# cvxopt/smcp

Measured on AMD Instinct MI355X. Metric: Newton KKT solves/sec, higher is better.
Workload: dtype f64; 1 GPU; synth50k nested block-arrow SDP n=50000, 8073 cliques, m=100; kktsolver=chol, n=50000, cliques=8073, m=100, blkval_doubles=2493568, update_doubles=10689536, parallelism=single

## Files before the change

smcp_amd/csrc/capi.hip:

```cpp
#include <hip/hip_runtime.h>
#include <memory>
#include <unordered_map>

#include <algorithm>
#include <chrono>
#include <cstdio>
#include <cstring>
#include <map>
#include <new>
#include <atomic>
#include <thread>
#include <type_traits>
#include <vector>

#include "../../include/smcp_amd.h"
#include "context.hpp"
#include "switches.hpp"
#include "front_generic.hip"
#include "front_mfma.hip"
#include "front_large.hip"
#include "front_inv.hip"
#include "front_n16.hip"
#include "front_fam.hip"
#include "front_fam2.hip"
#include "front_lfsp.hip"
#include "front_leafgram.hip"
#include "front_famt.hip"
#include "front_flow.hip"
#include "front_mrc.hip"
#include "front_edm.hip"

using namespace smcp;

#define HIPCHK(x)                                                                        \
  do {                                                                                   \
    hipError_t e_ = (x);                                                                 \
    if (e_ != hipSuccess) {                                                              \
      fprintf(stderr, "smcp_amd: HIP error %s at %s:%d\n", hipGetErrorString(e_), __FILE__, __LINE__); \
      return SMCP_EHIP;                                                                  \
    }                                                                                    \
  } while (0)

namespace {

enum {
  KID_chol_level = 0, KID_llt_level, KID_pinv_level, KID_gather_level, KID_completion_all,
  KID_hess_up_level, KID_hess_down_level, KID_hess_down_inv_all, KID_hess_up_inv_level, KID_scale_an,
  KID_factor_yaa, KID_trsm_fwd_level, KID_trsm_bwd_level, KID_amap, KID_aadj, KID_scatter_constraints,
  KID_dense_potrf, KID_dense_potrs, KID_vec_axpby, KID_axpby, KID_reduce_cliques, KID_reduce_final,
  KID_hess_up_mfma, KID_hess_down_mfma, KID_chol_mfma, KID_pinv_mfma, KID_prep_lk,
  KID_hess_up_mfma_hbm, KID_hess_down_mfma_hbm, KID_chol_mfma_hbm, KID_pinv_mfma_hbm,
  KID_gram_partial, KID_gram_reduce, KID_hess_up_pad,
  KID_lf_assemble, KID_lf_clear_upd, KID_lf_up1, KID_lf_up2, KID_lf_up3, KID_lf_down1, KID_lf_down2, KID_lf_down3,
  KID_lf_pinv1, KID_lf_pinv2, KID_lf_diag, KID_lf_chol_panel, KID_lf_chol_trail, KID_lf_pack_upd,
  KID_lf_prep_s, KID_lf_prep_row, KID_lf_prep_k, KID_factor_yaa_lds,
  KID_factor_inverse, KID_hess_down_inv_mfma, KID_hess_down_inv_mfma_hbm, KID_hess_up_inv_mfma, KID_hess_up_inv_mfma_hbm,
  KID_completion_mfma, KID_completion_mfma_hbm, KID_lf_copy_an, KID_lf_ri_an, KID_lf_dinv1, KID_lf_dinv2,
  KID_lf_uinv1, KID_lf_uinv2, KID_lf_completion, KID_hess_up_n16, KID_llt_mfma, KID_llt_mfma_hbm, KID_lf_llt,
  KID_hess_up_fam, KID_qr_rmul, KID_qr_dots, KID_qr_comb, KID_qr_small, KID_fam2_prep, KID_mid_chol, KID_lf_diag_inv, KID_lfsp_up, KID_lfsp_prep, KID_leaf_gram, KID_leaf_tables, KID_fam_sparse, KID_gram_diag128, KID_lf_assemble_lds, KID_fam_terms, KID_famt_prep, KID_lf_assemble_lds_dyn, KID_lf_zsp, KID_fam_terms_grp, KID_lf_assemble_fz, KID_factor_inverse_lds, KID_chol_flow,
  KID_mrc_diag, KID_mrc_rank, KID_mrc_reduce, KID_mrc_factor, KID_cut_signs, KID_cut_weights,
  KID_edm_rank, KID_edm_reduce, KID_edm_factor, KID_edm_dense,
  KID_COUNT
};
const char* const KID_NAMES[KID_COUNT] = {
  "k_chol_level", "k_llt_level", "k_pinv_level", "k_gather_level", "k_completion_all",
  "k_hess_up_level", "k_hess_down_level", "k_hess_down_inv_all", "k_hess_up_inv_level", "k_scale_an",
  "k_factor_yaa", "k_trsm_fwd_level", "k_trsm_bwd_level", "k_amap", "k_aadj", "k_scatter_constraints",
  "k_dense_potrf", "k_dense_potrs", "k_vec_axpby", "k_axpby", "k_reduce_cliques", "k_reduce_final",
  "k_hess_up_mfma<true>", "k_hess_down_mfma<true>", "k_chol_mfma<true>", "k_pinv_mfma<true>", "k_prep_lk",
  "k_hess_up_mfma<false>", "k_hess_down_mfma<false>", "k_chol_mfma<false>", "k_pinv_mfma<false>",
  "k_gram_partial", "k_gram_reduce", "k_hess_up_pad",
  "k_lf_assemble", "k_lf_clear_upd", "k_lf_up1", "k_lf_up2", "k_lf_up3", "k_lf_down1", "k_lf_down2", "k_lf_down3",
  "k_lf_pinv1", "k_lf_pinv2", "k_lf_diag", "k_lf_chol_panel", "k_lf_chol_trail", "k_lf_pack_upd",
  "k_lf_prep_s", "k_lf_prep_row", "k_lf_prep_k", "k_factor_yaa_lds",
  "k_factor_inverse", "k_hess_down_inv_mfma<true>", "k_hess_down_inv_mfma<false>", "k_hess_up_inv_mfma<true>",
  "k_hess_up_inv_mfma<false>", "k_completion_mfma<true>", "k_completion_mfma<false>", "k_lf_copy_an", "k_lf_ri_an",
  "k_lf_dinv1", "k_lf_dinv2", "k_lf_uinv1", "k_lf_uinv2", "k_lf_completion", "k_hess_up_n16",
  "k_llt_mfma<true>", "k_llt_mfma<false>", "k_lf_llt", "k_hess_up_fam",
  "k_stack_trsm", "k_stack_dots", "k_stack_comb", "k_qr_small", "k_fam2_prep", "k_mid_chol", "k_lf_diag_inv", "k_lfsp_up", "k_lfsp_prep", "k_leaf_pairs", "k_leaf_tables", "k_fam_sparse", "k_gram_diag128", "k_lf_assemble_lds", "k_fam_terms", "k_famt_prep", "k_lf_assemble_lds_dyn", "k_lf_zsp", "k_fam_terms_grp", "k_lf_assemble_fz", "k_factor_inverse_lds", "k_chol_flow",
  "k_mrc_diag", "k_mrc_rank", "k_mrc_reduce", "k_mrc_factor", "k_cut_signs", "k_cut_weights",
  "k_edm_rank", "k_edm_reduce", "k_edm_factor", "k_edm_dense"};

inline void note_launch(csp_ctx* c, int kid) {
  const hipError_t e = hipGetLastError();
  if (e != hipSuccess && !c->launch_err) {
    c->launch_err = (int)e;
    fprintf(stderr, "smcp_amd: launch of %s failed: %s\n", (kid >= 0 && kid < KID_COUNT) ? KID_NAMES[kid] : "?", hipGetErrorString(e));
  }
}
inline hipError_t end_call(csp_ctx* c) {
  hipError_t e = hipGetLastError();
  if (e == hipSuccess && c->launch_err) e = c->launch_err > 0 ? (hipError_t)c->launch_err : hipErrorLaunchFailure;
  c->launch_err = 0;
  return e;
}

__global__ void k_race_spin(long long ticks) {
  const long long t0 = wall_clock64();
  for (int it = 0; it < (1 << 22) && wall_clock64() - t0 < ticks; ++it) __builtin_amdgcn_s_sleep(8);
}
struct RaceInject {
  std::atomic<uint64_t> state{0};
  std::atomic<int64_t> injected{0};
  std::atomic<int> max_us{200};
  std::atomic<int> drop_joins{0};
  bool on() const { return state.load(std::memory_order_relaxed) != 0; }
  void seed(uint64_t s) { state.store(s ? (s * 0x9E3779B97F4A7C15ull) | 1ull : 0ull); }
  uint64_t next() {
    uint64_t x = state.load(std::memory_order_relaxed);
    x ^= x << 13; x ^= x >> 7; x ^= x << 17;
    state.store(x | 1ull, std::memory_order_relaxed);
    return x;
  }
};
inline RaceInject& race_inject() {
  static RaceInject r;
  static const bool init = [] { const char* e = sw_str("SMCP_RACE"); if (e && atoll(e) > 0) r.seed((uint64_t)atoll(e)); return true; }();
  (void)init;
  return r;
}
inline void race_delay(hipStream_t s, bool always = true) {
  RaceInject& r = race_inject();
  if (!r.on()) return;
  const uint64_t x = r.next();
  if (!always && (x >> 40) % 4 != 0) return;
  const long long us = 5 + (long long)((x >> 16) % (uint64_t)std::max(1, r.max_us.load(std::memory_order_relaxed) - 4));
  hipLaunchKernelGGL(k_race_spin, dim3(1), dim3(64), 0, s, us * 100);
  r.injected.fetch_add(1, std::memory_order_relaxed);
}

inline unsigned sync_event_flags() {
  static int sys = -1;
  if (sys < 0) { const char* e = sw_str("SMCP_EVENT_SYSFENCE"); sys = (e && e[0] == '1') ? 1 : 0; }
  return sys ? hipEventDisableTiming : (hipEventDisableTiming | hipEventReleaseToDevice);
}
struct Fork {
  csp_ctx* c; hipStream_t main; hipStream_t s; int which; bool on;
  static bool enabled() {
    static int e = -1;
    if (e < 0) { const char* v = sw_str("SMCP_FORK"); e = (v && v[0] == '0') ? 0 : 1; }
    return e == 1 && !trace_on_early();
  }
  static bool trace_on_early() { static const bool t = [] { const char* e = sw_str("SMCP_TRACE"); return e && e[0] == '1'; }(); return t; }
  Fork(csp_ctx* c_, hipStream_t st, int which_) : c(c_), main(st), s(st), which(which_), on(false) {
    if (!enabled()) return;
    if (!c->aux_fork && hipEventCreateWithFlags(&c->aux_fork, sync_event_flags()) != hipSuccess) { c->aux_fork = nullptr; return; }
    if (!c->aux_stream[which]) {
      static int prio = -2;
      if (prio == -2) { const char* e = sw_str("SMCP_AUX_PRIO"); prio = (e && e[0] == '0') ? 0 : 1; }
      int lo = 0, hi = 0;
      hipError_t rc = hipErrorUnknown;
      static int prio1 = -2;
      if (prio1 == -2) { const char* e = sw_str("SMCP_AUX_PRIO1"); prio1 = (e && e[0] == '0') ? 0 : 1; }
      if (which == 0 && prio && hipDeviceGetStreamPriorityRange(&lo, &hi) == hipSuccess && hi < lo)
        rc = hipStreamCreateWithPriority(&c->aux_stream[which], hipStreamNonBlocking, hi);
      if (which == 1 && prio1 && hipDeviceGetStreamPriorityRange(&lo, &hi) == hipSuccess && hi < lo)
        rc = hipStreamCreateWithPriority(&c->aux_stream[which], hipStreamNonBlocking, lo);
      if (rc != hipSuccess) rc = hipStreamCreateWithFlags(&c->aux_stream[which], hipStreamNonBlocking);
      if (rc != hipSuccess) { c->aux_stream[which] = nullptr; return; }
    }
    if (!c->aux_join[which] && hipEventCreateWithFlags(&c->aux_join[which], sync_event_flags()) != hipSuccess) { c->aux_join[which] = nullptr; return; }
    if (hipEventRecord(c->aux_fork, main) != hipSuccess) return;
    if (hipStreamWaitEvent(c->aux_stream[which], c->aux_fork, 0) != hipSuccess) return;
    s = c->aux_stream[which];
    on = true;
    if (race_inject().on()) {
      if (race_inject().drop_joins.load(std::memory_order_relaxed)) {
        hipLaunchKernelGGL(k_race_spin, dim3(1), dim3(64), 0, s, (long long)race_inject().max_us.load() * 100);
      } else race_delay((race_inject().next() >> 33) & 1 ? s : main);
    }
  }
  void join() {
    if (!on) return;
    on = false;
    if (race_inject().on() && ((race_inject().next() >> 33) & 1)) race_delay(s);
    if (race_inject().drop_joins.load(std::memory_order_relaxed)) { (void)hipEventRecord(c->aux_join[which], s); return; }
    if (hipEventRecord(c->aux_join[which], s) != hipSuccess || hipStreamWaitEvent(main, c->aux_join[which], 0) != hipSuccess)
      (void)hipStreamSynchronize(s);
  }
  ~Fork() { join(); }
};

inline bool trace_on() {
  static int t = -1;
  if (t < 0) { const char* e = sw_str("SMCP_TRACE"); t = (e && e[0] == '1') ? 1 : 0; }
  return t == 1;
}
inline void trace_launch(int kid, dim3 grid, dim3 block, size_t lds, hipStream_t st, bool before) {
  if (before) fprintf(stderr, "launch %s grid (%u,%u,%u) block %u lds %zu\n", KID_NAMES[kid], grid.x, grid.y, grid.z, block.x, lds);
  else (void)hipStreamSynchronize(st);
}
template <class K, class... A>
inline void launch_lds(csp_ctx* c, int kid, K kern, dim3 grid, dim3 block, size_t lds, hipStream_t st, A... args) {
  if (trace_on()) trace_launch(kid, grid, block, lds, st, true);
  Profiler& P = c->prof;
  const bool timed = P.want(kid);
  if (timed) (void)hipEventRecord(P.next(), st);
  race_delay(st, false);
  hipLaunchKernelGGL(kern, grid, block, lds, st, args...);
  note_launch(c, kid);
  if (trace_on()) trace_launch(kid, grid, block, lds, st, false);
  if (timed) {
    (void)hipEventRecord(P.next(), st);
    P.kids.push_back(kid);
  }
}
template <class K, class... A>
inline void launch(csp_ctx* c, int kid, K kern, dim3 grid, dim3 block, hipStream_t st, A... args) {
  if (trace_on()) trace_launch(kid, grid, block, 0, st, true);
  Profiler& P = c->prof;
  const bool timed = P.want(kid);
  if (timed) (void)hipEventRecord(P.next(), st);
  race_delay(st, false);
  hipLaunchKernelGGL(kern, grid, block, 0, st, args...);
  note_launch(c, kid);
  if (trace_on()) trace_launch(kid, grid, block, 0, st, false);
  if (timed) {
    (void)hipEventRecord(P.next(), st);
    P.kids.push_back(kid);
  }
}

template <class F>
void run_threads(int nth, F work) {
  if (nth <= 1) { work(0); return; }
  std::vector<std::thread> pool;
  int started = 0;
  try {
    for (; started < nth; ++started) pool.emplace_back(work, started);
  } catch (...) {
  }
  for (int tix = started; tix < nth; ++tix) work(tix);
  for (auto& th : pool) th.join();
}
// ... 1025 lines not shown
                          c->D.kc_ij && a0.ymode == 2 && a0.ysc && c->D.fam_maxterms <= FAMT_TCAP / 2 &&
                          c->D.cnnz <= (int64_t)4 * c->S.nsn * std::max<int64_t>(1, c->D.m);
  if (groups_on || fgroups_on) a0.chskip = groups_on && fgroups_on ? c->D.both_skip : (groups_on ? c->D.lfsp_skip : c->D.famt_skip);
  c->fz_live = false;
  {
    static int fzenv = -1;
    if (fzenv < 0) { const char* e = sw_str("SMCP_FZ"); fzenv = (e && e[0] == '0') ? 0 : 1; }
    bool want = fzenv && sparse && (set == 0 || (set == 1 && c->fz_set1_ok)) && lev_lo == 0 && lev_hi < 0 && !fgroups_on && c->D.fz_ok && !famt_disabled() && !fam2_disabled() &&
                c->D.lg_request && c->D.kc_ij && a0.ymode == 2 && a0.ysc && famt_terms_ok(c->D) &&
                c->D.cnnz <= (int64_t)4 * c->S.nsn * std::max<int64_t>(1, c->D.m) && !use_generic(c) && use_large() && c->D.gp_tptr;
    int famlevels = 0, nofill = 0;
    if (want) {
      for (int64_t l = 0; l < c->S.nlev; ++l)
        for_level_classes(c, l, a0, [&](bool lds, MfmaArgs a, int cnt, size_t, int) {
          if (lds && a.nS > 0 && a.level > 0) ++famlevels;
          if (!lds && (size_t)a.level < c->fz_levels.size() && c->fz_levels[(size_t)a.level] && !(a.nchmax > 0 && lf_assemble_fills(c, a, cnt, nrhs, true))) { want = false; ++nofill; }
        }, set);
      if (famlevels != 1) want = false;
    }
    if (want) { a0.fz_on = 1; a0.fz_no = c->D.fz_no; }
    static int occ = -1;
    if (occ < 0) occ = sw_on("SMCP_OCC", 0);
    if (occ && sparse)
      fprintf(stderr, "fz: want %d famlevels %d nofill %d nlev %d (env %d set %d lev %d..%d fgroups %d fz_ok %d famt_off %d fam2_off %d lg_request %d kc_ij %d ymode %d ysc %d maxterms %d cnnz %lld nsn %lld m %lld generic %d nrhs %d)\n",
              (int)want, famlevels, nofill, (int)c->S.nlev, fzenv, set, (int)lev_lo, (int)lev_hi, (int)fgroups_on, (int)c->D.fz_ok, (int)famt_disabled(), (int)fam2_disabled(), (int)c->D.lg_request,
              c->D.kc_ij != nullptr, a0.ymode, a0.ysc != nullptr, (int)c->D.fam_maxterms, (long long)c->D.cnnz, (long long)c->S.nsn, (long long)c->D.m, (int)use_generic(c), nrhs);
  }
  auto dense_input_on = [&](MfmaArgs& a, int cnt, double* Ub, int nr, hipStream_t s) {
    if (!sparse) return;
    for (int r0 = 0; r0 < nr; r0 += 65535) {
      MfmaArgs af = a;
      af.kc_j0 = a.kc_j0 + r0;
      const int64_t pan = (int64_t)(a.nnmax + a.namax) * a.nnmax;
      const int nz = (int)std::max<int64_t>(1, std::min<int64_t>(std::min<int64_t>(a.nnmax, 64), pan / 16384));
      launch(c, KID_scatter_constraints, k_panel_fill, dim3(cnt, std::min(65535, nr - r0), nz), dim3(256), s, af, Ub + (int64_t)r0 * ldu, ldu);
    }
    a.kc_ptr = nullptr;
  };
  auto dense_input = [&](MfmaArgs& a, int cnt) { dense_input_on(a, cnt, U, nrhs, st); };
  for (int64_t l = lev_lo; l < (lev_hi < 0 ? c->S.nlev : lev_hi); ++l) {
    for_level_classes(c, l, a0, [&](bool lds, MfmaArgs a, int cnt, size_t bytes, int thr) {
      static int fam_minrhs = -1;
      if (fam_minrhs < 0) { const char* e = sw_str("SMCP_FAM_MINRHS"); fam_minrhs = e ? atoi(e) : 1; }
      if (lds && a.nS > 0 && (sparse || nrhs >= fam_minrhs)) {
        const int nS = a.nS;
        a.nS = 0;
        if (a.level > 0) {
          MfmaArgs af = a;
          af.t.lev = a.t.lev + (cnt - nS);
          if (fgroups_on && (size_t)l < c->famt_grp.size() && c->famt_grp[(size_t)l].ngroups > 0) {
            af.grp_ptr = c->famt_grp[(size_t)l].ptr; af.grp_list = c->famt_grp[(size_t)l].list; af.famt_ngrp = c->famt_grp[(size_t)l].ngroups;
          }
          if (!try_fam(c, af, nS, nrhs, U, ldu, st)) {
            fprintf(stderr, "smcp_amd: family kernel not launchable (LDS budget or attribute)\n");
            if (!c->launch_err) c->launch_err = -1;
          }
        }
        cnt -= nS;
        if (cnt == 0) return;
      }
      int g = rhs_groups(cnt, nrhs, lds ? 2048 : 1024);
      if (lds) {
        hipStream_t ls = st;
        static int oldk = -1;
        if (oldk < 0) { const char* e = sw_str("SMCP_OLDLDS"); oldk = (e && e[0] == '1') ? 1 : 0; }
        size_t pbytes = (size_t)pad_layout(a.nnmax, a.namax, a.nchmax, a.panmax, a.pkmax, a.plansum).total * sizeof(double);
        if (!oldk && try_n16(c, a, cnt, nrhs, U, ldu, ls)) {
        } else if (!oldk && pbytes <= LDS_LIMIT) {
          dense_input_on(a, cnt, U, nrhs, ls);
          launch_lds(c, KID_hess_up_pad, k_hess_up_pad, dim3(cnt, g), dim3(pbytes > 48 * 1024 ? 512 : 256), pbytes, ls, a, U, ldu);
        } else {
          dense_input_on(a, cnt, U, nrhs, ls);
          launch_lds(c, KID_hess_up_mfma, k_hess_up_mfma<true>, dim3(cnt, g), dim3(thr), bytes, ls, a, U, ldu);
        }
      } else if (use_large() && c->D.gp_tptr) {
        {
          const csp_ctx::LfspGroups* grp = groups_on && (size_t)l < c->lfsp_grp.size() && c->lfsp_grp[(size_t)l].ngroups > 0 ? &c->lfsp_grp[(size_t)l] : nullptr;
          if (sparse && try_lfsp(c, a, cnt, nrhs, U, ldu, st, grp)) return;
          if (grp) {
            fprintf(stderr, "smcp_amd: sparse-input sweep of a grouped level not launchable\n");
            if (!c->launch_err) c->launch_err = -1;
          }
        }
        static int split_min = -1;
        if (split_min < 0) { const char* e = sw_str("SMCP_RHS_SPLIT"); split_min = e ? atoi(e) : 16; }
        static int parts = -1;
        if (parts < 0) { const char* e = sw_str("SMCP_RHS_PARTS"); parts = (e && e[0] == '3') ? 3 : 2; }
        const int ncu_split = c->D.ncu;
        static int dynsplit = -1;
        if (dynsplit < 0) { const char* e = sw_str("SMCP_ALDS_DYN"); const char* f = sw_str("SMCP_RHS_SPLIT_DYN"); dynsplit = ((e && e[0] == '0') || (f && f[0] == '1')) ? 1 : 0; }
        if (dynsplit && split_min > 0 && a.nchmax > 0 && nrhs >= split_min && (int64_t)cnt * nrhs > ncu_split && Fork::enabled()) {
          auto part = [&](int r0, int nr, hipStream_t s) {
            MfmaArgs ap = a;
            ap.nrhs = nr;
            ap.t.upd += (int64_t)r0 * a.t.updlen;
            ap.t.updp += (int64_t)r0 * a.t.updplen;
            ap.t.tmp += (int64_t)r0 * a.t.tmplen;
            ap.kc_j0 = a.kc_j0 + r0;
            dense_input_on(ap, cnt, U + (int64_t)r0 * ldu, nr, s);
            lf_up(c, ap, cnt, nr, U + (int64_t)r0 * ldu, ldu, s);
          };
          if (parts == 3 && nrhs >= 3) {
            const int h1 = nrhs / 3, h2 = (2 * nrhs) / 3;
            Fork f0(c, st, 0);
            part(h2, nrhs - h2, f0.s);
            Fork f1(c, st, 1);
            part(h1, h2 - h1, f1.s);
            part(0, h1, st);
            return;
          }
          const int h = nrhs / 2;
          Fork f(c, st, 0);
          part(h, nrhs - h, f.s);
          part(0, h, st);
          return;
        }
        static int zsp = -1;
        if (zsp < 0) { const char* e = sw_str("SMCP_ZSP"); zsp = (e && e[0] == '0') ? 0 : 1; }
        if (zsp && sparse && c->D.kc_sorted && a.nchmax == 0 && a.namax == 0 && lf_sym_split(a.nnmin) && a.nnmax <= LF_ZSP_MAXNN) {
          const int ntN = tiles64(a.nnmax);
          launch_lds(c, KID_lf_zsp, k_lf_zsp, dim3(a.nnmax, cnt, nrhs), dim3(256), (size_t)a.nnmax * sizeof(double), st, a, U, ldu);
          LAUNCH_PD(c, KID_lf_up2, k_lf_up2, dim3(umax1(ntN * (ntN + 1) / 2), cnt, nrhs), dim3(256), st, a, U, ldu);
          return;
        }
        const bool fzlev = c->fz_live && (size_t)a.level < c->fz_levels.size() && c->fz_levels[(size_t)a.level];
        if (sparse && a.nchmax > 0 && lf_assemble_fills(c, a, cnt, nrhs, fzlev)) {
          lf_up(c, a, cnt, nrhs, U, ldu, st, true);
          return;
        }
        dense_input(a, cnt);
        if (yroot && a.namax == 0 && a.nnmax <= ROOT_FUSED_MAXNN && root_fused()) {
          if (a.nchmax > 0) lf_assemble(c, a, cnt, nrhs, U, ldu, 0, st, true);
          const int ntN = tiles64(a.nnmax);
          LAUNCH_PD(c, KID_lf_up1, k_lf_root1, dim3(umax1(ntN * ntN), cnt, nrhs), dim3(256), st, a, U, ldu, yroot);
          return;
        }
        lf_up(c, a, cnt, nrhs, U, ldu, st);
      }
      else { dense_input(a, cnt); launch_lds(c, KID_hess_up_mfma_hbm, k_hess_up_mfma<false>, dim3(cnt, nrhs), dim3(thr), 0, st, a, U, ldu); }
    }, set);
  }
}
void gather_set(csp_ctx* c, int set, const double* x, int64_t ldx, int nrhs, double* updbase, hipStream_t st) {
  TreeArgs a = tree_args(c);
  const LevelSet& LS = c->sets[set];
  for (int64_t l = c->S.nlev - 1; l >= 0; --l) {
    const LevelClass& L = LS.lvl[l];
    const int cnt = (int)(L.nI + L.nII);
    if (!cnt) continue;
    a.lev = LS.lev2 + LS.off[l];
    launch(c, KID_gather_level, k_gather_level, dim3(cnt, nrhs, gather_parts(std::max(L.namaxI, L.namaxII), (int64_t)cnt * nrhs, c->D.ncu)), dim3(NT), st, a, x, ldx, updbase);
  }
}
void hess_down_fast(csp_ctx* c, double* U, int nrhs, int64_t ldu, const double* ysc, int ymode, hipStream_t st, int set = 0,
                    const double* yroot = nullptr) {
  MfmaArgs a0 = mfma_args(c, ysc, ymode, nrhs);
  for (int64_t l = c->S.nlev - 1; l >= 0; --l)
    for_level_classes(c, l, a0, [&](bool lds, MfmaArgs a, int cnt, size_t bytes, int thr) {
      int g = rhs_groups(cnt, nrhs, lds ? 2048 : 1024);
      if (lds) {
        static int dw = -1;
        if (dw < 0) { const char* e = sw_str("SMCP_DOWN_W"); dw = (e && e[0] == '0') ? 0 : 1; }
        if (dw && ymode == 0 && a.nnmax <= 16 && a.namax <= 64 && a.nnmax >= 1) {
          const int gw = rhs_groups((cnt + 3) / 4, nrhs, 4096);
          const dim3 grid((cnt + 3) / 4, gw), blk(256);
          switch ((std::max(a.namax, 1) + 15) / 16) {
            case 1: launch(c, KID_hess_down_mfma, k_hess_down_w<1>, grid, blk, st, a, U, ldu, cnt); break;
            case 2: launch(c, KID_hess_down_mfma, k_hess_down_w<2>, grid, blk, st, a, U, ldu, cnt); break;
            case 3: launch(c, KID_hess_down_mfma, k_hess_down_w<3>, grid, blk, st, a, U, ldu, cnt); break;
            default: launch(c, KID_hess_down_mfma, k_hess_down_w<4>, grid, blk, st, a, U, ldu, cnt); break;
          }
        } else
        if (ymode == 0) {
          const size_t b0 = (size_t)mfma_lds_doubles_for(WK_DOWN0, a.nnmax, a.namax) * sizeof(double);
          launch_lds(c, KID_hess_down_mfma, k_hess_down_mfma<true, WK_DOWN0>, dim3(cnt, g), dim3(b0 > 48 * 1024 ? 512 : 256), b0, st, a, U, ldu);
        } else
        launch_lds(c, KID_hess_down_mfma, k_hess_down_mfma<true>, dim3(cnt, g), dim3(thr), bytes, st, a, U, ldu);
      }
      else if (use_large() && yroot && a.namax == 0 && a.nnmax <= ROOT_FUSED_MAXNN && root_fused() && c->D.gp_tptr) {
        const int ntN = tiles64(a.nnmax);
        LAUNCH_PD(c, KID_lf_down3, k_lf_root2, dim3(umax1(ntN * (ntN + 1) / 2), cnt, nrhs), dim3(256), st, a, U, ldu, yroot);
      }
      else if (use_large() && (ymode == 0 || ymode == 3 || ymode == 2)) {
        if (ymode && a.namax) {
          const int mtA = tiles64(a.namax), ntN = tiles64(a.nnmax);
          LAUNCH_PD(c, KID_lf_ri_an, k_lf_ri_an, dim3(umax1(mtA * ntN), cnt, nrhs), dim3(256), st, a, U, ldu, ymode == 2 ? 1 : 0);
          launch(c, KID_lf_copy_an, k_lf_copy_an, dim3(umax1(std::min(64, (a.namax * a.nnmax + 255) / 256)), cnt, nrhs), dim3(256), st, a, U, ldu, 0);
        }
        MfmaArgs a2 = a;
        a2.ymode = 0; a2.ysc = nullptr;
        lf_down(c, a2, cnt, nrhs, U, ldu, st);
      }
      else launch_lds(c, KID_hess_down_mfma_hbm, k_hess_down_mfma<false>, dim3(cnt, nrhs), dim3(thr), 0, st, a, U, ldu);
    }, set);
}

void lf_factor_inverse(csp_ctx* c, const MfmaArgs& a, int cnt, hipStream_t st) {
  dim3 blk(256);
  for (int ib = 0; ib < a.namax; ib += LB) {
    launch_lds(c, KID_lf_diag, k_lf_diag, dim3(cnt), diag_blk(), LF_DIAG_LDS, st, a, (double*)nullptr, c->D.fac, 4, ib, 0);
    if (ib > 0) launch(c, KID_lf_prep_s, k_lf_prep_s, dim3(umax1(tiles64(ib)), cnt), blk, st, a, (const double*)c->D.fac, c->D.faci, ib, 4);
    launch(c, KID_lf_prep_row, k_lf_prep_row, dim3(umax1(tiles64(ib) + 1), cnt), blk, st, a, (const double*)c->D.fac, c->D.faci, ib, 4, 0);
  }
}

inline hipError_t zero_flag(csp_ctx* c, hipStream_t st) {
  const bool skip = c->lazy_status && c->flags_clean;
  c->flags_clean = false;
  return skip ? hipSuccess : hipMemsetAsync(c->D.info, 0, sizeof(int) * c->ntrial, st);
}
void complete_fac(csp_ctx* c, hipStream_t st) {
  if (!c->D.fac_partial) return;
  c->D.fac_partial = false;
  MfmaArgs a0 = mfma_args(c, nullptr, 0, 1);
  for_level_classes(c, 0, a0, [&](bool lds, MfmaArgs am, int cnt, size_t, int) {
    if (!lds || !am.namax || am.nS <= 0) return;
    am.t.lev = am.t.lev + (cnt - am.nS);
    const size_t bytes = ((size_t)padld(am.namax) * am.namax + 256 + 8) * sizeof(double);
    launch_lds(c, KID_factor_yaa_lds, k_factor_yaa_lds, dim3(am.nS), dim3(fact_threads(am, 256, 2)), bytes, st, am, (const double*)c->D.yaa, c->D.fac);
  });
}
int prepare_yaa(csp_ctx* c, const double* Y, bool need_fac, hipStream_t st, bool need_inv, bool allow_partial) {
  TreeArgs a = tree_args(c);
  const bool nocache = cache_off();
  if (need_inv) need_fac = true;
  if (need_fac && !allow_partial && c->D.fac_partial && c->D.fac_tag == Y && Y && !nocache) complete_fac(c, st);
  if (nocache || c->D.yaa_tag != Y || !Y) {
    gather_all(c, Y, 0, 1, c->D.yaa, st);
    c->D.yaa_tag = Y;
    c->D.fac_tag = c->D.faci_tag = nullptr;
    c->D.part_valid = false;
    if (Y) fp_record(c, 2, Y, st);
  } else if (int rc = fp_check(c, 2, Y, st)) return rc;
  const bool fast = !use_generic(c) && use_large();
  if (need_fac && c->D.fac_tag != Y) {
    if (fast) {
      MfmaArgs a0 = mfma_args(c, nullptr, 0, 1);
      for_all_large(c, a0, [&](MfmaArgs am, int cnt) {
        if (am.namax) launch(c, KID_axpby, k_copy_upd_blocks, dim3(cnt, umax1(std::min(64, (am.namax * am.namax + 1023) / 1024))), dim3(256), st,
                             am.t, (const double*)c->D.yaa, c->D.fac);
      });
      {
        Fork fl(c, st, 0);
        for_all_large(c, a0, [&](MfmaArgs am, int cnt) { if (am.namax) lf_factor_yaa(c, am, cnt, c->D.fac, fl.s); });
        Fork fs(c, st, 1);
        int turn = 0;
        for (int64_t l = 0; l < c->S.nlev; ++l)
          for_level_classes(c, l, a0, [&](bool lds, MfmaArgs am, int cnt, size_t, int) {
            if (!lds) return;
            size_t bytes = ((size_t)padld(am.namax) * am.namax + 256 + 8) * sizeof(double);
            if (am.namax) launch_lds(c, KID_factor_yaa_lds, k_factor_yaa_lds, dim3(cnt), dim3(fact_threads(am, 256, 2)), bytes, (turn++ & 1) ? fs.s : st, am, (const double*)c->D.yaa, c->D.fac);
          });
      }
    } else {
      launch(c, KID_factor_yaa, k_factor_yaa, dim3((int)c->S.nsn), dim3(NT), st, a, c->D.yaa, c->D.fac);
    }
    c->D.fac_tag = Y;
    c->D.fac_partial = false;
    c->D.faci_tag = nullptr;
    c->D.fac_gen++;
  }
  if (need_inv && c->D.faci_tag != Y) {
    if (fast) {
      a.lev = c->D.lev3idx;
      MfmaArgs a0 = mfma_args(c, nullptr, 0, 1);
      static const bool rd = sw_on("SMCP_FACI_LDS", true);
      bool all_lds = rd;
      if (rd)
        for (int64_t l = 0; l < c->S.nlev; ++l)
          for_level_classes(c, l, a0, [&](bool lds, MfmaArgs am, int, size_t, int) { if (lds && am.namax > 64) all_lds = false; });
      if (!c->D.nI_total) {
      } else if (!all_lds) {
        launch(c, KID_factor_inverse, k_factor_inverse, dim3((int)c->D.nI_total), dim3(256), st, a, (const double*)c->D.fac, c->D.faci);
      } else {
        for (int64_t l = 0; l < c->S.nlev; ++l)
          for_level_classes(c, l, a0, [&](bool lds, MfmaArgs am, int cnt, size_t, int) {
            if (!lds || !am.namax) return;
            if (am.namax <= 32)
              launch_lds(c, KID_factor_inverse_lds, k_factor_inverse_lds<33>, dim3(cnt), dim3(128), (2 * 33 * 32 + 256) * sizeof(double), st, am, (const double*)c->D.fac, c->D.faci);
            else
              launch_lds(c, KID_factor_inverse_lds, k_factor_inverse_lds<65>, dim3(cnt), dim3(256), (2 * 65 * 64 + 1024) * sizeof(double), st, am, (const double*)c->D.fac, c->D.faci);
          });
      }
      for_all_large(c, a0, [&](MfmaArgs am, int cnt) { if (am.namax) lf_factor_inverse(c, am, cnt, st); });
    } else {
      a.lev = c->D.levidx;
      launch(c, KID_factor_inverse, k_factor_inverse, dim3((int)c->S.nsn), dim3(256), st, a, (const double*)c->D.fac, c->D.faci);
    }
    c->D.faci_tag = Y;
  }
  return 0;
}

constexpr size_t INV_STATIC_LDS = 16 * 128 * sizeof(double);
constexpr int LF_INV_MIN_NN = 24;

void hess_down_inv_fast(csp_ctx* c, const double* L, double* U, int nrhs, int64_t ldu, int ymode, hipStream_t st) {
  gather_all(c, U, ldu, nrhs, c->D.upd, st);
  MfmaArgs a0 = mfma_args(c, c->D.faci, ymode, nrhs);
  a0.LK = L;
  dim3 blk(256);
  for (int64_t l = 0; l < c->S.nlev; ++l)
    for_level_classes(c, l, a0, [&](bool lds, MfmaArgs a, int cnt, size_t bytes, int thr) {
      if (lds) {
        int g = rhs_groups(cnt, nrhs, 2048);
        launch_lds(c, KID_hess_down_inv_mfma, k_hess_down_inv_mfma<true>, dim3(cnt, g), dim3(thr), bytes, st, a, U, ldu);
      } else if (!use_large()) {
        launch_lds(c, KID_hess_down_inv_mfma_hbm, k_hess_down_inv_mfma<false>, dim3(cnt, nrhs), dim3(thr), 0, st, a, U, ldu);
      }
    });
  if (use_large())
    for_all_large(c, a0, [&](MfmaArgs a, int cnt) {
      const int mtA = tiles64(a.namax), ntN = tiles64(a.nnmax);
      LAUNCH_PD(c, KID_lf_dinv1, k_lf_dinv1, dim3(umax1(mtA * ntN + ntN * ntN), cnt, nrhs), blk, st, a, U, ldu);
      LAUNCH_PD(c, KID_lf_dinv2, k_lf_dinv2, dim3(umax1(ntN * (ntN + 1) / 2 + mtA * ntN), cnt, nrhs), blk, st, a, U, ldu);
      if (ymode == 1 && a.namax) {
        LAUNCH_PD(c, KID_lf_ri_an, k_lf_ri_an, dim3(umax1(mtA * ntN), cnt, nrhs), blk, st, a, U, ldu, 1);
        launch(c, KID_lf_copy_an, k_lf_copy_an, dim3(umax1(std::min(64, (a.namax * a.nnmax + 255) / 256)), cnt, nrhs), blk, st, a, U, ldu, 0);
      }
    });
}
void hess_up_inv_fast(csp_ctx* c, const double* L, double* U, int nrhs, int64_t ldu, int ymode, hipStream_t st) {
  MfmaArgs a0 = mfma_args(c, c->D.faci, ymode, nrhs);
  a0.LK = L;
  dim3 blk(256);
  for (int64_t l = 0; l < c->S.nlev; ++l)
    for_level_classes(c, l, a0, [&](bool lds, MfmaArgs a, int cnt, size_t bytes, int thr) {
      if (lds) {
        int g = rhs_groups(cnt, nrhs, 2048);
        launch_lds(c, KID_hess_up_inv_mfma, k_hess_up_inv_mfma<true>, dim3(cnt, g), dim3(thr), bytes, st, a, U, ldu);
      } else if (use_large() && c->D.gp_tptr && a.nnmax >= LF_INV_MIN_NN) {
        const int mtA = tiles64(a.namax), ntN = tiles64(a.nnmax);
        const dim3 gcopy(umax1(std::min(64, (a.namax * a.nnmax + 255) / 256)), cnt, nrhs);
        if (ymode == 3 && a.namax) {
          LAUNCH_PD(c, KID_lf_ri_an, k_lf_ri_an, dim3(umax1(mtA * ntN), cnt, nrhs), blk, st, a, U, ldu, 1);
          launch(c, KID_lf_copy_an, k_lf_copy_an, gcopy, blk, st, a, U, ldu, 0);
        }
        LAUNCH_PD(c, KID_lf_uinv1, k_lf_uinv1, dim3(umax1(mtA * ntN + ntN * ntN), cnt, nrhs), blk, st, a, U, ldu);
        LAUNCH_PD(c, KID_lf_uinv2, k_lf_uinv2, dim3(umax1(mtA * (mtA + 1) / 2 + mtA * ntN + ntN * (ntN + 1) / 2), cnt, nrhs), blk, st, a, U, ldu);
        if (a.namax) launch(c, KID_lf_copy_an, k_lf_copy_an, gcopy, blk, st, a, U, ldu, 0);
        lf_assemble(c, a, cnt, nrhs, U, ldu, 1, st);
        if (a.namax) launch(c, KID_lf_pack_upd, k_lf_pack_upd, dim3(umax1(std::min(64, (a.namax * a.namax + 255) / 256)), cnt, nrhs), blk, st, a);
      } else {
        launch_lds(c, KID_hess_up_inv_mfma_hbm, k_hess_up_inv_mfma<false>, dim3(cnt, nrhs), dim3(thr), 0, st, a, U, ldu);
      }
    });
}
// ... 1628 lines not shown
```

smcp_amd/csrc/switches.hpp:

```cpp
#pragma once
#include <cstdio>
#include <cstdlib>
#include <cstring>
#include <string>

extern char** environ;

namespace smcp {

struct Switch { const char* name; const char* dflt; const char* doc; };

static const Switch SWITCHES[] = {
  {"SMCP_GENERIC", "0", "1: any-size fixed-order kernels of front_generic.hip for every tree operation (as CSP_TUNE_DETERMINISTIC)"},
  {"SMCP_LARGE", "1", "0: no tiled large-front kernels (fronts beyond LDS take the one-workgroup HBM kernels)"},
  {"SMCP_NOCACHE", "0", "1: nothing derived from (L, Y) is reused between calls"},
  {"SMCP_FORK", "1", "0: no side streams, everything on the caller's stream"},
  {"SMCP_AUX_PRIO", "1", "0: side stream 0 (few-workgroup chains) at default instead of highest priority"},
  {"SMCP_AUX_PRIO1", "1", "0: side stream 1 (filler work) at default instead of lowest priority"},
  {"SMCP_EVENT_SYSFENCE", "0", "1: internal events with the default system-scope release (12 us per hand-over instead of 7)"},
  {"SMCP_SCALING_OVERLAP", "1", "0: csp_cholesky_projected_inverse as its three steps one after the other"},
  {"SMCP_CHOL_PREP", "1", "0: k_prep_lk in a launch of its own instead of inside k_chol_mfma (narrow supernodes)"},
  {"SMCP_FAC_PARTIAL", "1", "0: chol(Y_AA) of the family children always formed by the fused scaling point"},
  {"SMCP_MID", "1", "0: per-step kernels instead of k_mid_chol / k_lf_diag_inv for fronts of at most 272 rows"},
  {"SMCP_TRTRI", "1", "0: block-row triangular inversion of large fronts instead of recursive doubling"},
  {"SMCP_N16", "1", "0: no shape-specialised k_hess_up_n16"},
  {"SMCP_OLDLDS", "0", "1: k_hess_up_mfma<true> instead of the padded / n16 kernels"},
  {"SMCP_DOWN_W", "1", "0: k_hess_down_mfma instead of the one-wave k_hess_down_w"},
  {"SMCP_FAM", "1", "0: no family kernels (per-level sweeps with the update exchange through HBM)"},
  {"SMCP_FAM2", "1", "0: no sparse-input family kernels (k_fam_sparse, k_fam_terms): k_hess_up_fam"},
  {"SMCP_FAMT", "1", "0: no entry-driven family sweep k_fam_terms (k_fam_sparse instead)"},
  {"SMCP_FZ", "1", "0: the family parents' packed updates go through HBM (k_fam_terms writes, the extend-add reads) instead of being formed by k_lf_assemble_fz"},
  {"SMCP_FAMT_GROUP", "1", "0: no sibling groups of family parents (k_fam_terms_grp)"},
  {"SMCP_LFSP", "1", "0: dense phases instead of the sparse-input sweep k_lfsp_up of childless large fronts"},
  {"SMCP_LFSP_GROUP", "1", "0: no sibling groups in k_lfsp_up"},
  {"SMCP_ZSP", "1", "0: dense first phase of wide childless fronts instead of k_lf_zsp"},
  {"SMCP_LEAFGRAM", "1", "0: never the closed-form Gram blocks of the family children (k_leaf_tables / k_leaf_pairs)"},
  {"SMCP_LG_SIDE", "1", "0: leaf Gram blocks after the sweep on the caller's stream instead of beside the top phases"},
  {"SMCP_GRAM_EARLY", "0", "1: the Gram chunks of the levels 0 / 1 rows on the side branch beside the top fronts' phase kernels (measured slower: 3.37 against 3.22 ms per step)"},
  {"SMCP_LG_EARLY", "1", "0: leaf Gram blocks beside the phase kernels of the top fronts instead of from the start of the sweep"},
  {"SMCP_FACI_LDS", "1", "0: inverse Y_AA factors of the small fronts by block rows against HBM (k_factor_inverse) instead of in LDS"},
  {"SMCP_FZ_TAIL", "1", "0: every (front, right-hand side) pair of the fused extend-add is one workgroup's task, also in a thin last round"},
  {"SMCP_GRAM", "1", "0: reference (two-sweep) formulation of the Schur complement instead of the Gram formulation"},
  {"SMCP_SCM", "1", "0: column-sparse constraints swept like the others (no SCMcolumn2 route)"},
  {"SMCP_TRSM_MM", "1", "0: csp_trsm through the generic level kernels instead of tile products"},
  {"SMCP_ALDS", "1", "0: extend-add of large fronts by gather plan only (no LDS streaming kernel)"},
  {"SMCP_ALDS_DYN", "1", "0: one workgroup per (front, right-hand side) instead of the task-drawing grid"},
  {"SMCP_ALDS_FILL", "1", "0: k_panel_fill builds the input panels instead of the extend-add (sgn 3)"},
  {"SMCP_ASM", "plan", "t: tiled extend-add kernel instead of the gather plan"},
  {"SMCP_ROOT_FUSED", "0", "1: fused two-product sweep of fronts without separator (Y_NN explicit: condition squared; studies only)"},
  {"SMCP_PD", "0", "1: four-wave tile products everywhere (no sixteen-wave shape for small launches)"},
  {"SMCP_POTRF_OLD", "0", "1: generic one-workgroup dense Cholesky"},
  {"SMCP_FLOW", "1", "0: no one-launch blocked Cholesky with in-launch tile dataflow (front_flow.hip): per-step kernels for dense matrices / single fronts beyond 272 rows"},
  {"SMCP_FLOW_WG", "112", "workgroups of that launch (at most 112: four launches fit the chip side by side)"},
  {"SMCP_POTRS_OLD", "0", "1: generic one-workgroup dense solve"},
  {"SMCP_POTRS_STEPS", "0", "1: per-block launches of the dense solve instead of k_dense_potrs_one"},
  {"SMCP_POTRF_DEFER", "1", "0: kkt_schur_factor factors H at once even under deferred status"},
  {"SMCP_QR_TRSM", "mfma", "f: vector-FMA substitution kernel of kkt_qr instead of the MFMA one"},
  {"SMCP_FTHR_CHOL", "128", "threads of k_chol_mfma on the leaf class"},
  {"SMCP_FTHR_PINV", "256", "threads of k_pinv_mfma on the leaf class"},
  {"SMCP_FTHR_YAA", "64", "threads of k_factor_yaa_lds on the leaf class"},
  {"SMCP_FTHR_YAA_MID", "256", "threads of k_factor_yaa_lds on separator blocks of 33 .. 64 rows"},
  {"SMCP_N16_THR_LEAF", "128", "threads of k_hess_up_n16 for one or two right-hand sides on childless fronts"},
  {"SMCP_DIAG_THREADS", "512", "threads of k_lf_diag"},
  {"SMCP_POTRF_THREADS", "1024", "threads of k_dense_potrf_small"},
  {"SMCP_FZ_THREADS", "1024", "threads of k_lf_assemble_fz (512: eight waves, no register spills, slower)"},
  {"SMCP_PD_WGS", "1", "largest launch, in workgroups per CU, that takes the sixteen-wave tile shape"},
  {"SMCP_ALDS_Z", "0", "workgroups per (front, right-hand side) of the LDS extend-add (0: automatic)"},
  {"SMCP_RHS_SPLIT", "16", "fewest right-hand sides for the two-stream split of a large-front sweep (plain extend-add launch only)"},
  {"SMCP_RHS_PARTS", "2", "parts of that split (2 or 3)"},
  {"SMCP_RHS_SPLIT_DYN", "0", "1: the split also with the task-drawing extend-add"},
  {"SMCP_FAM_MINRHS", "1", "fewest dense right-hand sides for the family kernel"},
  {"SMCP_FAMT_G", "0", "right-hand-side slices per family of k_fam_terms (0: cost model)"},
  {"SMCP_FAM2_STAG", "0", "stagger of k_fam_sparse's groups (studies)"},
  {"SMCP_FAMT_MEAN", "36", "entry-driven family sweeps (k_fam_terms, fused extend-add) up to this many entries per (family, constraint) list ON AVERAGE (lists up to 384 entries, in chunks); beyond: the dense family sweep"},
  {"SMCP_LFSP_OCC", "2", "waves per SIMD the grouped update phase of k_lfsp_up is compiled for (1: 512 registers, no spills; 2: 256, ~100 spilled)"},
  {"SMCP_LFSP_G", "1", "right-hand sides per workgroup of k_lfsp_up"},
  {"SMCP_GRAM_NW", "16", "waves per workgroup of k_gram_diag128 (4, 8 or 16)"},
  {"SMCP_GRAM_MINCHUNK", "512", "fewest stack rows per workgroup of the Gram accumulation"},
  {"SMCP_UPDP_PAD", "0", "doubles of padding between the packed exchange buffers of consecutive right-hand sides"},
  {"SMCP_QR_PASSES", "0", "Cholesky-QR passes of kkt_qr (0: decided by the deviation test)"},
  {"SMCP_QR_P", "1", "positions per lane of the FMA substitution kernel (1 or 2)"},
  {"SMCP_FLOW_STAMPS", "0", "1: per-workgroup time accounts of the one-launch blocked Cholesky on stderr (waits for every launch)"},
  {"SMCP_POISON", "0", "1: every fp64 device buffer of the library (and the exchange buffers of smcp_amd/kkt.py) starts as 4.5e150 (hunting reads of never-written workspace)"},
  {"SMCP_RACE", "0", "seed > 0: delay injection on every internal stream hand-over and one launch in eight (race hunting; results must not change)"},
  {"SMCP_TRACE", "0", "1: every launch named on stderr and waited for (a device fault points at its kernel)"},
  {"SMCP_TIMING", "0", "1: wall-clock marks of the set-up phases on stderr"},
  {"SMCP_OCC", "0", "1: occupancy decisions of k_hess_up_n16 on stderr"},
  {"SMCP_DEBUG_ADDR", "0", "1: addresses of the large allocations on stderr"},
  {"SMCP_CONTIG", "0", "1: large buffers from physically contiguous memory (placement studies: slower)"},
  {"SMCP_SKIP", "0", "phase mask of the sweep kernels (ablation timing; results are wrong)"},
  {"SMCP_GSKIP", "0", "ablation mask of the Gram kernel (results are wrong)"},
  {"SMCP_LGSKIP", "0", "ablation mask of k_leaf_pairs (results are wrong)"},
  {"SMCP_QR_FAKE", "0", "1: timing experiment of the FMA substitution kernel (results are wrong)"},
};

inline void sw_check_environment() {
  static const bool done = [] {
    for (char** e = environ; e && *e; ++e) {
      if (std::strncmp(*e, "SMCP_", 5) != 0) continue;
      const char* eq = std::strchr(*e, '=');
      const std::string name(*e, eq ? (size_t)(eq - *e) : std::strlen(*e));
      if (name.rfind("SMCP_BENCH_", 0) == 0 || name.rfind("SMCP_FUZZ_", 0) == 0 || name == "SMCP_CXXFLAGS" || name == "SMCP_STAMPS" ||
          name == "SMCP_SHARD_KEEP" || name == "SMCP_SHARD_TOP" || name == "SMCP_GIT_SHA" || name == "SMCP_FS_MODE") continue;
      bool known = false;
      for (const Switch& s : SWITCHES) if (name == s.name) known = true;
      if (!known) std::fprintf(stderr, "smcp_amd: unknown switch %s in the environment (see smcp_amd/csrc/switches.hpp)\n", name.c_str());
    }
    return true;
  }();
  (void)done;
}
inline const char* sw_str(const char* name) {
  sw_check_environment();
  bool known = false;
  for (const Switch& s : SWITCHES) if (!std::strcmp(name, s.name)) { known = true; break; }
  if (!known) std::fprintf(stderr, "smcp_amd: switch %s is read but not listed in switches.hpp\n", name);
  return std::getenv(name);
}
inline int sw_on(const char* name, int dflt) { const char* v = sw_str(name); return v ? (v[0] == '0' ? 0 : (v[0] == '1' ? 1 : dflt)) : dflt; }
inline int sw_int(const char* name, int dflt) { const char* v = sw_str(name); return v ? std::atoi(v) : dflt; }

}
```

Baseline: 320.3 KKT solves/s.

## Fuse family parent and children down-sweep into one LDS-resident kernel

Adds k_hess_down_fam, which processes a family parent and up to eight of its children in one workgroup during the root-to-leaves Hessian down sweep. The parent's packed front stays in LDS so the children read it without a round trip through HBM, and the level-1 families are deferred so they can be merged with the level-0 lone fronts into a single launch. The aim is to cut per-level launches and global-memory traffic for the many small fronts. In exchange it adds a large templated kernel whose LDS footprint depends on the largest front, and it only applies when nrhs is at most the SMCP_DOWN_FAM limit (default 1) and ymode is 0.

```diff
diff --git a/smcp_amd/csrc/capi.hip b/smcp_amd/csrc/capi.hip
--- a/smcp_amd/csrc/capi.hip
+++ b/smcp_amd/csrc/capi.hip
@@ -21,6 +21,7 @@
 #include "front_large.hip"
 #include "front_inv.hip"
 #include "front_n16.hip"
+#include "front_downfam.hip"
 #include "front_fam.hip"
 #include "front_fam2.hip"
 #include "front_lfsp.hip"
@@ -59,7 +60,7 @@
   KID_lf_uinv1, KID_lf_uinv2, KID_lf_completion, KID_hess_up_n16, KID_llt_mfma, KID_llt_mfma_hbm, KID_lf_llt,
   KID_hess_up_fam, KID_qr_rmul, KID_qr_dots, KID_qr_comb, KID_qr_small, KID_fam2_prep, KID_mid_chol, KID_lf_diag_inv, KID_lfsp_up, KID_lfsp_prep, KID_leaf_gram, KID_leaf_tables, KID_fam_sparse, KID_gram_diag128, KID_lf_assemble_lds, KID_fam_terms, KID_famt_prep, KID_lf_assemble_lds_dyn, KID_lf_zsp, KID_fam_terms_grp, KID_lf_assemble_fz, KID_factor_inverse_lds, KID_chol_flow,
   KID_mrc_diag, KID_mrc_rank, KID_mrc_reduce, KID_mrc_factor, KID_cut_signs, KID_cut_weights,
-  KID_edm_rank, KID_edm_reduce, KID_edm_factor, KID_edm_dense,
+  KID_edm_rank, KID_edm_reduce, KID_edm_factor, KID_edm_dense, KID_hess_down_fam,
   KID_COUNT
 };
 const char* const KID_NAMES[KID_COUNT] = {
@@ -79,7 +80,7 @@
   "k_llt_mfma<true>", "k_llt_mfma<false>", "k_lf_llt", "k_hess_up_fam",
   "k_stack_trsm", "k_stack_dots", "k_stack_comb", "k_qr_small", "k_fam2_prep", "k_mid_chol", "k_lf_diag_inv", "k_lfsp_up", "k_lfsp_prep", "k_leaf_pairs", "k_leaf_tables", "k_fam_sparse", "k_gram_diag128", "k_lf_assemble_lds", "k_fam_terms", "k_famt_prep", "k_lf_assemble_lds_dyn", "k_lf_zsp", "k_fam_terms_grp", "k_lf_assemble_fz", "k_factor_inverse_lds", "k_chol_flow",
   "k_mrc_diag", "k_mrc_rank", "k_mrc_reduce", "k_mrc_factor", "k_cut_signs", "k_cut_weights",
-  "k_edm_rank", "k_edm_reduce", "k_edm_factor", "k_edm_dense"};
+  "k_edm_rank", "k_edm_reduce", "k_edm_factor", "k_edm_dense", "k_hess_down_fam"};
 
 inline void note_launch(csp_ctx* c, int kid) {
   const hipError_t e = hipGetLastError();
@@ -1411,11 +1412,51 @@
     launch(c, KID_gather_level, k_gather_level, dim3(cnt, nrhs, gather_parts(std::max(L.namaxI, L.namaxII), (int64_t)cnt * nrhs, c->D.ncu)), dim3(NT), st, a, x, ldx, updbase);
   }
 }
+int down_fam_maxrhs() {
+  static int v = -1;
+  if (v < 0) v = std::min(65535, std::max(0, sw_int("SMCP_DOWN_FAM", 1)));
+  return v;
+}
+void launch_down_fam(csp_ctx* c, const MfmaArgs& a, int cnt, int nrhs, double* U, int64_t ldu, hipStream_t st,
+                     const int32_t* lone = nullptr, int nlone = 0, int lnn = 0, int lna = 0) {
+  const int nfmax = std::max(a.famnn + a.famna, lnn + lna), cpan = (a.famcnn + a.famcna) * a.famcnn;
+  const size_t bytes = down_fam_lds_bytes(nfmax, cpan);
+  const int pnat = (std::max(std::max(a.famna, lna), 1) + 15) / 16, cnat = (std::max(a.famcna, 1) + 15) / 16;
+  const dim3 grid(cnt + nlone, nrhs), blk(256);
+  switch (2 * pnat + cnat) {
+    case 3: launch_lds(c, KID_hess_down_fam, k_hess_down_fam<1, 1>, grid, blk, bytes, st, a, U, ldu, nfmax, cpan, cnt, lone); break;
+    case 4: launch_lds(c, KID_hess_down_fam, k_hess_down_fam<1, 2>, grid, blk, bytes, st, a, U, ldu, nfmax, cpan, cnt, lone); break;
+    case 5: launch_lds(c, KID_hess_down_fam, k_hess_down_fam<2, 1>, grid, blk, bytes, st, a, U, ldu, nfmax, cpan, cnt, lone); break;
+    case 6: launch_lds(c, KID_hess_down_fam, k_hess_down_fam<2, 2>, grid, blk, bytes, st, a, U, ldu, nfmax, cpan, cnt, lone); break;
+    case 7: launch_lds(c, KID_hess_down_fam, k_hess_down_fam<3, 1>, grid, blk, bytes, st, a, U, ldu, nfmax, cpan, cnt, lone); break;
+    case 8: launch_lds(c, KID_hess_down_fam, k_hess_down_fam<3, 2>, grid, blk, bytes, st, a, U, ldu, nfmax, cpan, cnt, lone); break;
+    case 9: launch_lds(c, KID_hess_down_fam, k_hess_down_fam<4, 1>, grid, blk, bytes, st, a, U, ldu, nfmax, cpan, cnt, lone); break;
+    default: launch_lds(c, KID_hess_down_fam, k_hess_down_fam<4, 2>, grid, blk, bytes, st, a, U, ldu, nfmax, cpan, cnt, lone); break;
+  }
+}
 void hess_down_fast(csp_ctx* c, double* U, int nrhs, int64_t ldu, const double* ysc, int ymode, hipStream_t st, int set = 0,
                     const double* yroot = nullptr) {
   MfmaArgs a0 = mfma_args(c, ysc, ymode, nrhs);
+  MfmaArgs fam1 = a0;
+  int nfam1 = 0;
   for (int64_t l = c->S.nlev - 1; l >= 0; --l)
     for_level_classes(c, l, a0, [&](bool lds, MfmaArgs a, int cnt, size_t bytes, int thr) {
+      if (lds && a.nS > 0 && ymode == 0 && nrhs <= down_fam_maxrhs()) {
+        const int nS = a.nS;
+        a.nS = 0;
+        MfmaArgs af = a;
+        af.t.lev = a.t.lev + (cnt - nS);
+        cnt -= nS;
+        if (a.level > 1) launch_down_fam(c, af, nS, nrhs, U, ldu, st);
+        else if (a.level == 1) { fam1 = af; nfam1 = nS; }
+        else if (nfam1 > 0) {
+          const bool fits = cnt > 0 && a.nnmax <= 16 && a.namax <= 64;
+          launch_down_fam(c, fam1, nfam1, nrhs, U, ldu, st, fits ? a.t.lev : nullptr, fits ? cnt : 0, fits ? a.nnmax : 0, fits ? a.namax : 0);
+          nfam1 = 0;
+          if (fits) return;
+        }
+        if (cnt == 0) return;
+      }
       int g = rhs_groups(cnt, nrhs, lds ? 2048 : 1024);
       if (lds) {
         static int dw = -1;
@@ -1452,6 +1493,7 @@
       }
       else launch_lds(c, KID_hess_down_mfma_hbm, k_hess_down_mfma<false>, dim3(cnt, nrhs), dim3(thr), 0, st, a, U, ldu);
     }, set);
+  if (nfam1 > 0) launch_down_fam(c, fam1, nfam1, nrhs, U, ldu, st);
 }
 
 void lf_factor_inverse(csp_ctx* c, const MfmaArgs& a, int cnt, hipStream_t st) {
diff --git a/smcp_amd/csrc/front_downfam.hip b/smcp_amd/csrc/front_downfam.hip
--- /dev/null
+++ b/smcp_amd/csrc/front_downfam.hip
@@ -0,0 +1,256 @@
+#include <hip/hip_runtime.h>
+
+namespace smcp {
+
+__device__ inline int pk_low(int hi, int lo, int n) { return hi + ((lo * (2 * n - lo - 1)) >> 1); }
+__host__ inline size_t down_fam_lds_bytes(int nfmax, int cpan) { return (size_t)(nfmax * (nfmax + 1) / 2 + 4 * (2 * cpan + 16)) * sizeof(double); }
+
+template <int M>
+struct DownOps {
+  double li[4], kk[4 * M], g[4], q[4 * M];
+  int ri[M], rj[4 * M];
+};
+
+template <int NAT, int M>
+__device__ inline void down_fam_load_lk(double (&li)[4], double (&kk)[4 * M], const double* LK, const CliqueDesc& d, int lane) {
+  const int l15 = lane & 15, kq = lane >> 4;
+  const int nn = d.nn, na = d.na, nf = nn + na;
+#pragma unroll
+  for (int s = 0; s < 4; ++s) {
+    const int r = kq + 4 * s;
+    const double v = LK[(unsigned)(min(r, nn - 1) + min(l15, nn - 1) * nf)];
+    li[s] = (r < nn && l15 < nn && r >= l15) ? v : 0.0;
+  }
+#pragma unroll
+  for (int s = 0; s < 4 * NAT; ++s) {
+    const int j = kq + 4 * s;
+    const double v = LK[(unsigned)((na > 0 ? nn + min(j, na - 1) : 0) + min(l15, nn - 1) * nf)];
+    kk[s] = (j < na && l15 < nn) ? v : 0.0;
+  }
+}
+
+struct DownStage { double* P; double* LK; int32_t* rel; };
+__device__ inline DownStage down_fam_stage_of(double* base, int wave, int cpan) {
+  double* w = base + (size_t)wave * (2 * cpan + 16);
+  return DownStage{w, w + cpan, (int32_t*)(w + 2 * cpan)};
+}
+__device__ inline void down_fam_stage(const DownStage& st, const MfmaArgs& a, const CliqueDesc& d, const double* U, int lane) {
+  const int pan = (d.nn + d.na) * d.nn;
+  const double* P = U + d.blk;
+  const double* LK = a.LK + d.blk;
+  for (int e0 = 0; e0 < pan; e0 += 256) {
+    double vp[4], vl[4];
+#pragma unroll
+    for (int h = 0; h < 4; ++h) {
+      const int e = e0 + 64 * h + lane;
+      vp[h] = e < pan ? P[(unsigned)e] : 0.0;
+      vl[h] = e < pan ? LK[(unsigned)e] : 0.0;
+    }
+#pragma unroll
+    for (int h = 0; h < 4; ++h) {
+      const int e = e0 + 64 * h + lane;
+      if (e < pan) { st.P[e] = vp[h]; st.LK[e] = vl[h]; }
+    }
+  }
+  if (lane < d.na) st.rel[lane] = a.t.relidx[d.rel + lane];
+  __builtin_amdgcn_wave_barrier();
+}
+
+template <int NAT, int M>
+__device__ inline void down_fam_load(DownOps<M>& o, const DownStage& st, const CliqueDesc& d, int lane) {
+  const int l15 = lane & 15, kq = lane >> 4;
+  const int nn = d.nn, na = d.na, nf = nn + na;
+  down_fam_load_lk<NAT, M>(o.li, o.kk, st.LK, d, lane);
+#pragma unroll
+  for (int t = 0; t < NAT; ++t) o.ri[t] = st.rel[min(16 * t + l15, na - 1)];
+#pragma unroll
+  for (int s = 0; s < 4 * NAT; ++s) o.rj[s] = st.rel[min(kq + 4 * s, na - 1)];
+#pragma unroll
+  for (int s = 0; s < 4; ++s) {
+    const int c = kq + 4 * s;
+    const int hi = min(max(l15, c), nn - 1), lo = min(min(l15, c), nn - 1);
+    const double v = st.P[hi + lo * nf];
+    o.g[s] = (l15 < nn && c < nn) ? v : 0.0;
+  }
+#pragma unroll
+  for (int t = 0; t < NAT; ++t) {
+    const int m = 16 * t + l15;
+#pragma unroll
+    for (int s = 0; s < 4; ++s) {
+      const int c = kq + 4 * s;
+      const double v = st.P[nn + min(m, na - 1) + min(c, nn - 1) * nf];
+      o.q[4 * t + s] = (m < na && c < nn) ? v : 0.0;
+    }
+  }
+  __builtin_amdgcn_wave_barrier();
+}
+
+template <int NAT, bool OWN, int M>
+__device__ inline void down_fam_sweep(const DownOps<M>& o, const CliqueDesc& d, double* P, double* zs, int nfz, int lane) {
+  const int l15 = lane & 15, kq = lane >> 4;
+  const int nn = d.nn, na = d.na, nf = nn + na;
+  const d4 zero4 = {0.0, 0.0, 0.0, 0.0};
+  d4 tt = zero4, z1 = zero4;
+#pragma unroll
+  for (int s = 0; s < 4; ++s) {
+    double g = o.g[s];
+    if (OWN) {
+      const int c = kq + 4 * s;
+      const int hi = min(max(l15, c), nn - 1), lo = min(min(l15, c), nn - 1);
+      const double v = zs[pk_low(hi, lo, nfz)];
+      g = (l15 < nn && c < nn) ? v : 0.0;
+    }
+    tt = __builtin_amdgcn_mfma_f64_16x16x4f64(g, o.li[s], tt, 0, 0, 0);
+  }
+#pragma unroll
+  for (int s = 0; s < 4; ++s) z1 = __builtin_amdgcn_mfma_f64_16x16x4f64(o.li[s], tt[s], z1, 0, 0, 0);
+  d4 w = zero4;
+#pragma unroll
+  for (int t = 0; t < NAT; ++t) {
+    if (16 * t < na) {
+      double q[4];
+      const int m = 16 * t + l15, mc = min(m, na - 1);
+#pragma unroll
+      for (int s = 0; s < 4; ++s) {
+        q[s] = o.q[OWN ? s : 4 * t + s];
+        if (OWN) {
+          const int c = kq + 4 * s;
+          const double v = zs[pk_low(nn + mc, min(c, nn - 1), nfz)];
+          q[s] = (m < na && c < nn) ? v : 0.0;
+        }
+      }
+      d4 qlt = zero4, zkt = zero4;
+#pragma unroll
+      for (int s = 0; s < 4; ++s) qlt = __builtin_amdgcn_mfma_f64_16x16x4f64(q[s], o.li[s], qlt, 0, 0, 0);
+#pragma unroll
+      for (int s0 = 0; s0 < 4 * NAT; s0 += 8) {
+        double z[8];
+#pragma unroll
+        for (int s = s0; s < s0 + 8 && s < 4 * NAT; ++s) {
+          const int j = kq + 4 * s;
+          const int i1 = OWN ? nn + mc : o.ri[t], j1 = OWN ? nn + min(j, na - 1) : o.rj[s];
+          const double v = zs[pk_low(max(i1, j1), min(i1, j1), nfz)];
+          z[s - s0] = (m < na && j < na) ? v : 0.0;
+        }
+#pragma unroll
+        for (int s = s0; s < s0 + 8 && s < 4 * NAT; ++s) zkt = __builtin_amdgcn_mfma_f64_16x16x4f64(z[s - s0], o.kk[s], zkt, 0, 0, 0);
+        if (4 * NAT > 8) __builtin_amdgcn_sched_barrier(0);
+      }
+      d4 dt;
+#pragma unroll
+      for (int rr = 0; rr < 4; ++rr) {
+        dt[rr] = qlt[rr] - 0.5 * zkt[rr];
+        const int mm = 16 * t + kq + 4 * rr;
+        if (mm < na && l15 < nn) {
+          const double v = qlt[rr] - zkt[rr];
+          P[nn + mm + l15 * nf] = v;
+          if (OWN) zs[pk_low(nn + mm, l15, nfz)] = v;
+        }
+      }
+#pragma unroll
+      for (int s = 0; s < 4; ++s) {
+        w = __builtin_amdgcn_mfma_f64_16x16x4f64(dt[s], o.kk[4 * t + s], w, 0, 0, 0);
+        w = __builtin_amdgcn_mfma_f64_16x16x4f64(o.kk[4 * t + s], dt[s], w, 0, 0, 0);
+      }
+      __builtin_amdgcn_sched_barrier(0);
+    }
+  }
+#pragma unroll
+  for (int rr = 0; rr < 4; ++rr) {
+    const int c = kq + 4 * rr;
+    if (l15 < nn && c <= l15) {
+      const double v = z1[rr] - w[rr];
+      P[l15 + (int64_t)c * nf] = v;
+      if (OWN) zs[pk_low(l15, c, nfz)] = v;
+    }
+  }
+}
+
+template <int PNAT, int CNAT>
+__global__ void __launch_bounds__(256, 4) k_hess_down_fam(MfmaArgs a, double* u, int64_t ldu, int nfmax, int cpan, int nfam, const int32_t* lone) {
+  extern __shared__ double zs[];
+  const int lane = threadIdx.x & 63;
+  const int wave = __builtin_amdgcn_readfirstlane((int)(threadIdx.x >> 6));
+  const int k = (int)blockIdx.x < nfam ? a.t.lev[blockIdx.x] : lone[(int)blockIdx.x - nfam];
+  const CliqueDesc d = a.t.cl[k];
+  const int nn = d.nn, na = d.na, nf = nn + na;
+  const int nch = (int)blockIdx.x < nfam ? d.chend - d.chbeg : 0;
+  double* U = u + (int64_t)blockIdx.y * ldu;
+  double* P = U + d.blk;
+  const int q0 = (wave + 3) & 3;
+  const bool has0 = q0 < nch, has1 = q0 + 4 < nch;
+  const CliqueDesc dc0 = a.t.cl[has0 ? a.t.chidx[d.chbeg + q0] : k];
+  const CliqueDesc dc1 = a.t.cl[has1 ? a.t.chidx[d.chbeg + q0 + 4] : k];
+  const DownStage st = down_fam_stage_of(zs + nfmax * (nfmax + 1) / 2, wave, cpan);
+  constexpr int M = PNAT > CNAT ? PNAT : CNAT;
+  DownOps<M> o;
+  if (has0) down_fam_stage(st, a, dc0, U, lane);
+  if (wave == 0) down_fam_load_lk<PNAT, M>(o.li, o.kk, a.LK + d.blk, d, lane);
+  else if (has0) {
+    down_fam_load<CNAT, M>(o, st, dc0, lane);
+    if (has1) down_fam_stage(st, a, dc1, U, lane);
+  }
+  {
+    double v[8];
+#pragma unroll
+    for (int c = 0; c < 4; ++c) {
+      const int j = wave + 4 * c;
+#pragma unroll
+      for (int h = 0; h < 2; ++h) {
+        const int i = j + lane + 64 * h;
+        v[2 * c + h] = (j < nn && i < nf) ? P[i + j * nf] : 0.0;
+      }
+    }
+#pragma unroll
+    for (int c = 0; c < 4; ++c) {
+      const int j = wave + 4 * c;
+#pragma unroll
+      for (int h = 0; h < 2; ++h) {
+        const int i = j + lane + 64 * h;
+        if (j < nn && i < nf) zs[pk_low(i, j, nf)] = v[2 * c + h];
+      }
+    }
+  }
+  __builtin_amdgcn_sched_barrier(0);
+  if (na > 0) {
+    const bool haspar = d.parent >= 0;
+    const CliqueDesc par = a.t.cl[haspar ? d.parent : k];
+    const int nng = par.nn, nag = par.na, nfg = nng + nag;
+    const double* Pg = U + par.blk;
+    const double* Ug = a.t.upd + (int64_t)blockIdx.y * a.t.updlen + par.upd;
+    const int32_t* rel = a.t.relidx + d.rel;
+    const int gi = rel[min(lane, na - 1)];
+    double v[4 * PNAT];
+#pragma unroll
+    for (int c = 0; c < 4 * PNAT; ++c) {
+      const int j = wave + 4 * c;
+      v[c] = 0.0;
+      if (haspar && j < na && lane >= j && lane < na) {
+        const int gj = rel[j];
+        const int hi = max(gi, gj), lo = min(gi, gj);
+        v[c] = lo < nng ? Pg[hi + lo * nfg] : Ug[(hi - nng) + (lo - nng) * nag];
+      }
+    }
+#pragma unroll
+    for (int c = 0; c < 4 * PNAT; ++c) {
+      const int j = wave + 4 * c;
+      if (j < na && lane >= j && lane < na) zs[pk_low(nn + lane, nn + j, nf)] = v[c];
+    }
+  }
+  __syncthreads();
+  if (wave == 0) down_fam_sweep<PNAT, true, M>(o, d, P, zs, nf, lane);
+  __syncthreads();
+  if (has0) {
+    if (wave == 0) {
+      down_fam_load<CNAT, M>(o, st, dc0, lane);
+      if (has1) down_fam_stage(st, a, dc1, U, lane);
+    }
+    down_fam_sweep<CNAT, false, M>(o, dc0, U + dc0.blk, zs, nf, lane);
+  }
+  if (has1) {
+    down_fam_load<CNAT, M>(o, st, dc1, lane);
+    down_fam_sweep<CNAT, false, M>(o, dc1, U + dc1.blk, zs, nf, lane);
+  }
+}
+
+}
diff --git a/smcp_amd/csrc/switches.hpp b/smcp_amd/csrc/switches.hpp
--- a/smcp_amd/csrc/switches.hpp
+++ b/smcp_amd/csrc/switches.hpp
@@ -26,6 +26,7 @@
   {"SMCP_N16", "1", "0: no shape-specialised k_hess_up_n16"},
   {"SMCP_OLDLDS", "0", "1: k_hess_up_mfma<true> instead of the padded / n16 kernels"},
   {"SMCP_DOWN_W", "1", "0: k_hess_down_mfma instead of the one-wave k_hess_down_w"},
+  {"SMCP_DOWN_FAM", "1", "most right-hand sides of a root -> leaves sweep that take the one-launch family kernel k_hess_down_fam (0: never; the per-level k_hess_down_w launches)"},
   {"SMCP_FAM", "1", "0: no family kernels (per-level sweeps with the update exchange through HBM)"},
   {"SMCP_FAM2", "1", "0: no sparse-input family kernels (k_fam_sparse, k_fam_terms): k_hess_up_fam"},
   {"SMCP_FAMT", "1", "0: no entry-driven family sweep k_fam_terms (k_fam_sparse instead)"},
```

Measured after the change: 326.7 KKT solves/s, median of 6. 1.02x the previous value.
